# Hansard-T/FHE-Linformer

Hardware: AMD Instinct MI355X
Metric: encrypted Linformer-d128 forward ms/sample (lower is better)
Workload: dtype u64

## Files before the change

fhe-linformer_amd/csrc/context.cpp:

```cpp
#include "context.h"
#include <hip/hip_runtime.h>
#include <algorithm>
#include <cstdio>
#include <cstdlib>
#include <cstring>
#include <sys/random.h>
#include <time.h>
#include <cxxabi.h>
#include <dlfcn.h>
#include <execinfo.h>

namespace fhelin {

void hip_check(hipError_t e, const char* what) {
    if (e != hipSuccess) throw Error(FHELIN_ERR_HIP, std::string(what) + ": " + hipGetErrorString(e));
}

void* DevicePool::raw_malloc(size_t bytes) {
    if (backend_.malloc_fn) return backend_.malloc_fn(bytes);
    void* p = nullptr;
    if (hipMalloc(&p, bytes) != hipSuccess) {
        (void)hipGetLastError();
        return nullptr;
    }
// ... 279 lines not shown
            hip_check(hipStreamCreateWithFlags(&lane_stream[k], hipStreamNonBlocking), "hipStreamCreate(lane)");
            hip_check(hipEventCreateWithFlags(&lane_event[k], hipEventDisableTiming), "hipEventCreate(lane)");
        }
        hip_check(hipEventCreateWithFlags(&fork_event, hipEventDisableTiming), "hipEventCreate(fork)");
        pool.lane_stream[0] = main_stream;
        for (int k = 1; k <= n_lanes; ++k) pool.lane_stream[k] = lane_stream[k];
        pool.have_streams = true;
        if (const char* e = std::getenv("FHELIN_ASYNC")) async_lanes = std::atoi(e) != 0;
        if (const char* e = std::getenv("FHELIN_FUSE_MODDOWN")) fuse_moddown = std::atoi(e) != 0;
        if (const char* e = std::getenv("FHELIN_FUSE_FINISH")) fuse_finish = std::atoi(e) != 0;
        if (const char* e = std::getenv("FHELIN_HOST_ENCODE")) host_encode = std::atoi(e) != 0;
        if (const char* e = std::getenv("FHELIN_FUSE_GATHER")) fuse_gather = std::atoi(e) != 0;
        if (const char* e = std::getenv("FHELIN_ROT_GATHER")) rot_gather = std::atoi(e) != 0;
        if (const char* e = std::getenv("FHELIN_FUSE_LIFT")) fuse_lift = std::atoi(e) != 0;
        if (const char* e = std::getenv("FHELIN_LDS_DIGITS")) lds_digits = std::atoi(e) != 0;
        if (const char* e = std::getenv("FHELIN_NTT_TRACE")) trace_small_ntt = std::atoi(e);
        if (const char* e = std::getenv("FHELIN_SCALAR_TRACE")) trace_scalar = std::atoi(e);
        if (const char* e = std::getenv("FHELIN_HOST_WAITS")) trace_waits = std::atoi(e) != 0;
    }
    hip_check(hipEventCreate(&ev_start), "hipEventCreate");
    stage_words = (size_t)2 << p.log_n;
    for (int i = 0; i < STAGE_SLOTS; ++i) {
        hip_check(hipHostMalloc(reinterpret_cast<void**>(&stage_buf[i]), stage_words * sizeof(u64), hipHostMallocDefault), "hipHostMalloc(stage)");
        hip_check(hipEventCreateWithFlags(&stage_ev[i], hipEventDisableTiming), "hipEventCreate(stage)");
    }
    hip_check(hipHostMalloc(reinterpret_cast<void**>(&small_buf), (size_t)SMALL_SLOTS * SMALL_WORDS * sizeof(u64), hipHostMallocDefault), "hipHostMalloc(stage, small)");
    for (int i = 0; i < SMALL_SLOTS; ++i) hip_check(hipEventCreateWithFlags(&small_ev[i], hipEventDisableTiming), "hipEventCreate(stage, small)");
    hip_check(hipEventCreate(&ev_stop), "hipEventCreate");
    has_device = true;

// ... 375 lines not shown
```

fhe-linformer_amd/csrc/context.h:

```cpp
#pragma once
#include <cstdint>
#include <map>
#include <memory>
#include <stdexcept>
#include <string>
#include <unordered_map>
#include <vector>
#include <hip/hip_runtime_api.h>
#include "../../include/fhelin.h"
#include "hostmath.h"
#include "kernels.h"

namespace fhelin {

struct Params {
    int log_n = 16;
    int n_q = 24;
    int first_bits = 55;
    int scale_bits = 52;
    int n_p = 6;
    int special_bits = 60;
    int dnum = 4;
    int log_slots = 14;
    int hamming = 192;
// ... 204 lines not shown
    int limb_id_p(int j) const { return L + 1 + j; }
    int digits_at(int ell) const { return (ell + alpha - 1) / alpha; }
    u64 galois_element(int rot_index) const;
    const u32* automorph_map(u64 galois);
    const u32* automorph_inverse_of(const u32* map);
    std::map<const u32*, const u32*> automorph_inverse;
    u32 automorph_ginv_of(const u32* map) const;
    std::map<const u32*, u32> automorph_ginv;
    bool fuse_finish = true;
    bool fuse_moddown = false;
    bool host_encode = false;
    bool fuse_gather = true;
    bool rot_gather = true;
    bool fuse_lift = true;
    bool lds_digits = true;
    struct FftDev {
        const u32* rot = nullptr;
        const double* ksi = nullptr;
    };
    std::map<int, FftDev> fft_dev;
    void sync();
    void ntt(const LimbBatch& b, bool inverse, int active = -1) {
        stats.limb_ntt += (u64)(active >= 0 ? active : b.nvec);
        if (trace_small_ntt && b.nvec <= trace_small_ntt) note_small_ntt(b.nvec);
        launch_ntt(dt, b, inverse, stream);
    }
    bool trace_waits = false;
    std::map<std::string, std::pair<u64, u64>> wait_sites;
    void note_wait(const char* site, u64 ns) {
        auto& e = wait_sites[site];
// ... 18 lines not shown
```

fhe-linformer_amd/csrc/evaluator.cpp:

```cpp
#include "evaluator.h"
#include <map>
#include <hip/hip_runtime.h>
#include <cmath>
#include <cstring>

namespace fhelin {

DevBlock::~DevBlock() {
    if (d && ctx) {
        try { ctx->pool.free(d); } catch (...) {}
    }
}
Ciphertext::~Ciphertext() {
    if (async_ev) (void)hipEventDestroy(async_ev);
    if (d && ctx && !block) {
        try { ctx->pool.free(d); } catch (...) {}
    }
}
Encoding::~Encoding() {
    if (ready) (void)hipEventDestroy(ready);
    if (d && ctx) {
        try { ctx->pool.free(d, lanes_ordered); } catch (...) {}
    }
}
EvalKey::~EvalKey() {
    if (d && ctx) {
        try { ctx->pool.free(d); } catch (...) {}
    }
    if (d_perm && ctx) {
        try { ctx->pool.free(d_perm); } catch (...) {}
    }
}

static void launch_ok(const char* what) { hip_check(hipGetLastError(), what); }

CtPtr Evaluator::new_ct(int npoly, int ell, int deg, long double scale, int slots) {
    c_.require_device();
    if (ell < 1 || ell > c_.L + 1 || npoly < 1 || npoly > 3) throw Error(FHELIN_ERR_ARG, "new_ct: bad shape");
    auto ct = std::make_shared<Ciphertext>();
    ct->ctx = &c_;
    ct->npoly = npoly;
    ct->ell = ell;
    ct->deg = deg;
    ct->scale = scale;
    ct->slots = slots;
// ... 100 lines not shown
    if (rows) {
        sh.per_row = 1;
        sh.shared_input = shared ? 1 : 0;
        for (int b = 0; b < B; ++b) {
            sh.evk_row[b] = rows->keys[b]->d;
            sh.map_row[b] = rows->maps[b];
        }
    }
    KsShape shu = sh;
    shu.batch = shared ? 1 : B;
    c_.stats.keyswitch += (u64)B;
    c_.stats.keyswitch_limbs += (u64)B * ell;
    const bool identity = !map && !rows;
    const bool gather = !identity && !add1 && rot_in_gather();
    const u64* evk = key ? key->d : nullptr;
    if (gather) {
        sh.gather = 1;
        if (rows) {
            for (int b = 0; b < B; ++b) {
                sh.evk_row[b] = permuted(*rows->keys[b], rows->maps[b]);
                sh.ginv_row[b] = c_.automorph_ginv_of(rows->maps[b]);
            }
        } else {
            evk = permuted(*key, map);
            sh.map_row[0] = map;
            sh.ginv = c_.automorph_ginv_of(map);
        }
        if (add0) {
            sh.gsrc = add0;
            sh.gsrc_stride = add_stride;
// ... 130 lines not shown
        if (!rot_keys.count(c_.galois_element(r))) return false;
    }
    return !indices.empty();
}

const u64* Evaluator::permuted(const EvalKey& key, const u32* map) {
    if (key.d_perm) return key.d_perm;
    const int nvec = key.digits * 2 * (c_.L + 1 + c_.K);
    key.d_perm = c_.dalloc<u64>(key.words());
    launch_automorph_pack30(c_.dt, key.d_perm, key.d, map, nvec, c_.stream);
    launch_ok("key permutation");
    hip_check(hipStreamSynchronize(c_.stream), "key permutation sync");
    return key.d_perm;
}

std::vector<CtPtr> Evaluator::rotate_sum_batch(const std::vector<CtPtr>& vin, const std::vector<int>& indices) {
    if (vin.empty()) return {};
    const int R = (int)indices.size();
    if (R < 1 || R > KsShape::MAX_ROT) throw Error(FHELIN_ERR_ARG, "rotate_sum_batch: 1..7 rotations");
    if (!have_rotation_keys(indices, vin[0]->slots)) throw Error(FHELIN_ERR_KEY, "rotate_sum_batch: missing rotation key");
    if (c_.K < 1) throw Error(FHELIN_ERR_STATE, "hybrid key switching needs at least one special prime");
    std::vector<const EvalKey*> keys;
    std::vector<const u32*> maps;
    for (int r : indices) {
        const u64 g = c_.galois_element(r);
        keys.push_back(rot_keys.at(g).get());
        maps.push_back(c_.automorph_map(g));
    }
    const size_t N = c_.N;
    const int K = c_.K, L1 = c_.L + 1;
// ... 7 lines not shown
        for (size_t i = first; i < vin.size() && (int)idx.size() < batch_limit; ++i) {
            const CtPtr &a = vin[first], &b = vin[i];
            if (!done[i] && b->npoly == 2 && b->ell == a->ell && b->deg == a->deg && fabsl(b->scale / a->scale - 1.0L) < 1e-9L)
                idx.push_back(i);
        }
        std::vector<CtPtr> chunk;
        for (size_t i : idx) chunk.push_back(vin[i]);
        chunk = make_contiguous(chunk, 0);
        const int B = (int)chunk.size(), ell = chunk[0]->ell;
        const size_t pn = (size_t)ell * N, ctw = 2 * pn;
        const LevelTables& lt = c_.lvl[ell];
        std::vector<CtPtr> o = new_ct_batch(B, 2, ell, chunk[0]->deg, chunk[0]->scale, chunk[0]->slots);
        const u64* base = chunk[0]->d;
        KsShape sh{ell, K, c_.alpha, lt.beta, L1, B, ctw, ctw, pn, ctw};
        sh.n_rot = R;
        sh.lds_digits = c_.lds_digits ? 1 : 0;
        for (int r = 0; r < R; ++r) {
            sh.evk_rot[r] = permuted(*keys[r], maps[r]);
            sh.map_rot[r] = maps[r];
            if (c_.galois_element(indices[r]) % (u64)(c_.N / 256) != 1) sh.lds_digits = 0;
        }
        int steps = 0;
        while ((1 << steps) < R + 1) ++steps;
        c_.stats.keyswitch += (u64)B * steps;
        c_.stats.keyswitch_limbs += (u64)B * steps * ell;
        {
            Scratch<u64> ext = modup(sh, base + pn, false);
            Scratch<u64> accQ = c_.scratch<u64>((size_t)B * 2 * ell * N);
            Scratch<u64> accP = c_.scratch<u64>((size_t)B * 2 * K * N);
            const bool rp = sum_in_row_pass();
            if (c_.fuse_gather) {
// ... 100 lines not shown
        }
        std::vector<CtPtr> chunk;
        for (size_t i : idx) chunk.push_back(x[i]);
        chunk = make_contiguous(chunk, 0);
        const int B = (int)chunk.size(), ell = chunk[0]->ell;
        const size_t pn = (size_t)ell * N, ctw = 2 * pn;
        const LevelTables& lt = c_.lvl[ell];
        const long double sf = c_.sf_real[chunk[0]->level()];
        const bool merged = rescale_out && ell >= 2 && K + 1 <= 16;
        if (rescale_out && !merged) throw Error(FHELIN_ERR_STATE, "hoisted_dot_rows: no limb left to drop");
        const int oell = merged ? ell - 1 : ell;
        std::vector<CtPtr> o = new_ct_batch(B, 2, oell, merged ? chunk[0]->deg : chunk[0]->deg + 1, chunk[0]->scale * sf, chunk[0]->slots);
        const u64* base = chunk[0]->d;
        KsShape sh{ell, K, c_.alpha, lt.beta, L1, B, ctw, (size_t)2 * oell * N, pn, ctw};
        sh.n_rot = R;
        sh.lds_digits = c_.lds_digits ? 1 : 0;
        HoistAdd h;
        h.n_rot = R;
        std::vector<FoldedKey> hold;
        const std::shared_ptr<Encoding> e0 = pts[0]->at(ell, sf);
        h.v[0] = e0->d;
        for (int r = 0; r < R; ++r) {
            hold.push_back(folded_key(pts[r + 1], indices[r], sf));
            sh.evk_rot[r] = hold.back().d->d;
            sh.map_rot[r] = maps[r];
            h.v[r + 1] = hold.back().enc->d;
            h.map[r] = maps[r];
            if (c_.galois_element(indices[r]) % (u64)(c_.N / 256) != 1) sh.lds_digits = 0;
        }
        c_.stats.keyswitch += (u64)B * R;
        c_.stats.keyswitch_limbs += (u64)B * R * ell;
// ... 1054 lines not shown
            sadj = make_contiguous(sadj, 7);
        }
        ScalarSet cst;
        if (cadd != 0.0) real_to_scalars(c_, (long double)cadd * sc, ell, cst);
        KsShape sh{ell, K, c_.alpha, lt.beta, L1, B, 3 * pn, (size_t)2 * (ell - 1) * N, pn, 0};
        c_.stats.keyswitch += (u64)B;
        c_.stats.keyswitch_limbs += (u64)B * ell;
        c_.stats.rescale += (u64)B;
        c_.stats.rescale_limbs += (u64)B * ell;
        const u64* c_ntt = d[0]->d + 2 * pn;
        std::vector<CtPtr> o = new_ct_batch(B, 2, ell - 1, 1, 0, x[first]->slots);
        {
            Scratch<u64> ext = modup(sh, c_ntt, true);
            Scratch<u64> accQ = c_.scratch<u64>((size_t)B * 2 * ell * N);
            Scratch<u64> accP = c_.scratch<u64>((size_t)B * 2 * K * N);
            launch_ks_inner(c_.dt, sh, accQ, accP, ext, relin_key->d, c_ntt, s);
            launch_affine_acc(c_.dt, sh, accQ, d[0]->d, sadj.empty() ? nullptr : sadj[0]->d, cst, cadd != 0.0 ? 1 : 0, f, c_.d_pmod, s);
            if (f == 2) launch_ew_add(c_.dt, accP, accP, accP, B * 2 * K, B * 2 * K, L1, K, s);
            moddown_rescale(sh, accQ, accP, o[0]->d);
            launch_ok("mult_affine_rescale_batch");
        }
        for (int k = 0; k < B; ++k) {
            const size_t i = idx[k];
            o[k]->scale = x[i]->scale * y[i]->scale / (long double)c_.chain.q[ell - 1];
            out[i] = o[k];
            done[i] = 1;
        }
    }
    return out;
}

// ... 98 lines not shown
        }
        Scratch<u64> dcst = c_.scratch<u64>(cst.size());
        if (items.cst) c_.upload_async(dcst, cst.data(), cst.size());
        KsShape sh{ell, K, c_.alpha, c_.lvl[ell].beta, L1, B, 3 * pn, (size_t)2 * (ell - 1) * N, pn, 0};
        sh.accp_limbs = K + 1;
        c_.stats.keyswitch += (u64)B;
        c_.stats.keyswitch_limbs += (u64)B * ell;
        c_.stats.rescale += (u64)B;
        c_.stats.rescale_limbs += (u64)B * ell;
        const u64* c_ntt = d[0]->d + 2 * pn;
        std::vector<CtPtr> o = new_ct_batch(B, 2, ell - 1, 1, 0, x[first]->slots);
        {
            Scratch<u64> ext = modup(sh, c_ntt, true);
            Scratch<u64> accQ = c_.scratch<u64>((size_t)B * 2 * ell * N);
            Scratch<u64> accP = c_.scratch<u64>((size_t)B * 2 * (K + 1) * N);
            launch_ks_inner(c_.dt, sh, accQ, accP, ext, relin_key->d, c_ntt, s);
            launch_affine_acc_items(c_.dt, sh, items, accQ, accP, d[0]->d, dcst, c_.d_pmod, s);
            moddown_rescale_exact(sh, accQ, accP, o[0]->d, items.f2);
            launch_ok("mult_affine_batch");
        }
        for (int k = 0; k < B; ++k) {
            const size_t i = idx[k];
            o[k]->scale = x[i]->scale * y[i]->scale / (long double)c_.chain.q[ell - 1];
            out[i] = o[k];
            done[i] = 1;
        }
    }
    return out;
}

std::vector<CtPtr> Evaluator::add_plain_batch(const std::vector<CtPtr>& v, const PtPtr& p) {
    std::vector<CtPtr> out(v.size());
// ... 391 lines not shown
```

fhe-linformer_amd/csrc/evaluator.h:

```cpp
#pragma once
#include <functional>
#include <map>
#include <memory>
#include <vector>
#include "context.h"
#include "kernels_elem.h"

namespace fhelin {

struct DevBlock {
    Context* ctx = nullptr;
    u64* d = nullptr;
    ~DevBlock();
};

struct Ciphertext {
    Context* ctx = nullptr;
    u64* d = nullptr;
    std::shared_ptr<DevBlock> block;
    int npoly = 2;
    int ell = 0;
    int deg = 1;
    long double scale = 0;
    int slots = 0;
// ... 30 lines not shown
    std::vector<double> imag;
    int slots = 0;
    int level = 0;
    static constexpr size_t MAX_ENCODINGS = 16;
    std::vector<std::shared_ptr<Encoding>> cache;
    std::shared_ptr<Encoding> at(int ell, long double scale);
    std::shared_ptr<Plaintext> shared;
    static constexpr size_t MAX_SHARED_ENCODINGS = 64;
};
typedef std::shared_ptr<Plaintext> PtPtr;

struct EvalKey {
    Context* ctx = nullptr;
    u64* d = nullptr;
    mutable u64* d_perm = nullptr;
    int digits = 0;
    bool seeded = false;
    ~EvalKey();
    size_t words() const { return (size_t)digits * 2 * (ctx->L + 1 + ctx->K) * ctx->N; }
};
typedef std::shared_ptr<EvalKey> KeyPtr;

void real_to_scalars(const Context& c, long double v, int ell, ScalarSet& sc);

class Evaluator {
public:
    explicit Evaluator(Context& c) : c_(c) {}
    Context& ctx() { return c_; }

    CtPtr new_ct(int npoly, int ell, int deg, long double scale, int slots);
// ... 16 lines not shown

    void keyswitch(const u64* c_ntt, int ell, const EvalKey& key, u64* out, const u64* add0, const u64* add1, const u32* map,
                   const u64* post = nullptr);
    void keyswitch_batch(int batch, const u64* c_ntt, size_t c_stride, int ell, const EvalKey& key, u64* out, size_t out_stride,
                         const u64* add0, const u64* add1, size_t add_stride, const u32* map, const u64* post, size_t post_stride);
    struct KsRows {
        std::vector<const EvalKey*> keys;
        std::vector<const u32*> maps;
        bool shared_input = false;
    };
    void keyswitch_rows(const KsRows& rows, const u64* c_ntt, size_t c_stride, int ell, u64* out, size_t out_stride, const u64* add0,
                        size_t add_stride);
    std::vector<CtPtr> rotate_sum_batch(const std::vector<CtPtr>& v, const std::vector<int>& indices);
    bool have_rotation_keys(const std::vector<int>& indices, int slots) const;
    const u64* permuted(const EvalKey& key, const u32* map);
    CtPtr rotate_each_sum(const std::vector<CtPtr>& v, const std::vector<int>& indices);
    std::vector<CtPtr> rotate_each_sum_rows(const std::vector<std::vector<CtPtr>>& rows, const std::vector<int>& indices);
    std::vector<CtPtr> hoisted_dot_rows(const std::vector<CtPtr>& xs, const std::vector<PtPtr>& pts, const std::vector<int>& indices,
                                        bool rescale_out = false);
    bool merged_products = false;
    bool merged_rescale = true;
    bool double_hoist = true;
    struct FoldedKey {
        PtPtr pt;
        KeyPtr key;
        int index = 0;
        long double scale = 0;
        std::shared_ptr<Encoding> enc;
        std::shared_ptr<DevBlock> d;
    };
// ... 101 lines not shown
```

fhe-linformer_amd/csrc/kernels_elem.h:

```cpp
#pragma once
#include "kernels.h"

namespace fhelin {

struct ScalarSet {
    u64 v[128];
};

void launch_ew_mul(const DeviceTables& t, u64* out, const u64* a, const u64* b, int nvec, int b_mod, int limb_first, int limb_count, hipStream_t s);
void launch_ew_add(const DeviceTables& t, u64* out, const u64* a, const u64* b, int nvec, int b_mod, int limb_first, int limb_count, hipStream_t s);
void launch_ew_sub(const DeviceTables& t, u64* out, const u64* a, const u64* b, int nvec, int b_mod, int limb_first, int limb_count, hipStream_t s);
void launch_ew_muladd(const DeviceTables& t, u64* out, const u64* acc, const u64* a, const u64* b, int nvec, int b_mod, int limb_first,
                      int limb_count, hipStream_t s);
void launch_ew_neg(const DeviceTables& t, u64* out, const u64* a, int nvec, int limb_first, int limb_count, hipStream_t s);
void launch_ew_scalar(const DeviceTables& t, u64* out, const u64* a, const ScalarSet& sc, int nvec, int limb_first, int limb_count, hipStream_t s,
                      int in_limbs = 0);
void launch_ew_addscalar(const DeviceTables& t, u64* out, const u64* a, const ScalarSet& sc, int nvec, int limb_first, int limb_count, hipStream_t s,
                         int add_vecs = -1);
struct LinComb {
    static constexpr int MAX_TERMS = 32;
    int n = 0;
    int vecs = 0;
    const u64* a[MAX_TERMS];
};
// ... 101 lines not shown
    int n_rot = 0;
    const u64* evk_rot[MAX_ROT] = {};
    const u32* map_rot[MAX_ROT] = {};
    size_t rot_ext_stride = 0;
    size_t rot_input_stride = 0;
    int lds_digits = 0;
    size_t ext_batch_stride = 0;
    const u64* gsrc = nullptr;
    size_t gsrc_stride = 0;
    const u64* gsrc_pmod = nullptr;
    int gather = 0;
    u32 ginv = 0;
    u32 ginv_row[MAX_ROWS] = {};
    int tch = 16;
    int accp_limbs = 0;
};
void launch_modup_conv(const DeviceTables& t, const KsShape& sh, u64* ext, const u64* cc, const u64* c_ntt, const u64* hatinv,
                       const u64* hatmod, hipStream_t s);
void launch_ks_inner(const DeviceTables& t, const KsShape& sh, u64* accQ, u64* accP, const u64* ext, const u64* evk, const u64* c_ntt,
                     hipStream_t s);
void launch_ks_inner_multi(const DeviceTables& t, const KsShape& sh, u64* accQ, u64* accP, const u64* ext, const u64* c_ntt,
                           hipStream_t s);
void launch_fold_key(const DeviceTables& t, u64* out, const u64* key, const u32* map, const u64* V, int nvec, hipStream_t s);
struct HoistAdd {
    int n_rot = 0;
    const u64* v[KsShape::MAX_ROT + 1] = {};
    const u32* map[KsShape::MAX_ROT] = {};
    u64* acc = nullptr;
    const u64* pmod = nullptr;
};
void launch_hoist_addends(const DeviceTables& t, const KsShape& sh, const HoistAdd& h, u64* pre, const u64* ct, hipStream_t s);
void launch_gather_sum(const DeviceTables& t, const KsShape& sh, u64* out, const u64* in, size_t in_stride, hipStream_t s);
void launch_moddown_conv(const DeviceTables& t, const KsShape& sh, u64* conv, const u64* accP, const u64* phatinv, const u64* phatmod,
                         hipStream_t s);
void launch_affine_acc(const DeviceTables& t, const KsShape& sh, u64* accQ, const u64* d, const u64* sub, const ScalarSet& cst, int has_cst, int f,
                       const u64* pmod, hipStream_t s);
void launch_moddown_rescale_conv(const DeviceTables& t, const KsShape& sh, u64* conv, const u64* accP, const u64* top, const u64* hatinv,
                                 const u64* hatmod, const u64* mmod, hipStream_t s);
void launch_moddown_rescale_finish(const DeviceTables& t, const KsShape& sh, u64* out, const u64* accQ, const u64* conv, const u64* minv,
                                   hipStream_t s);
struct AffineItems {
    static constexpr int MAX_ITEMS = 32;
    const u64* add[MAX_ITEMS] = {};
    u32 f2 = 0, neg = 0, cst = 0;
};
void launch_affine_acc_items(const DeviceTables& t, const KsShape& sh, const AffineItems& it, u64* accQ, u64* accP, const u64* d,
                             const u64* consts, const u64* pmod, hipStream_t s);
void launch_moddown_rescale_exact_conv(const DeviceTables& t, const KsShape& sh, u32 f2, u64* conv, const u64* accP, const u64* phatinv,
                                       const u64* phatmod, const u64* pinv, const u64* pmod, const u64* qlm, hipStream_t s);
void launch_moddown_finish(const DeviceTables& t, const KsShape& sh, u64* out, const u64* accQ, const u64* conv, const u64* pinv,
                           const u64* add0, const u64* add1, const u32* map, const u64* post, hipStream_t s);

}
```

fhe-linformer_amd/csrc/kernels_ks.hip:

```cpp
#include <hip/hip_runtime.h>
#include <cstdlib>
#include "kernels.h"
#include "kernels_elem.h"

namespace fhelin {
namespace {

typedef u64 u64x2 __attribute__((ext_vector_type(2)));

__device__ __forceinline__ Barrett load_barrett(const DeviceTables& t, int limb) {
    Barrett b;
    b.q = t.moduli[limb];
    b.r0 = t.barrett[2 * limb];
    b.r1 = t.barrett[2 * limb + 1];
    return b;
}

constexpr int TCH = 16;

template <int MAXA, bool FULL>
__device__ __forceinline__ void modup_body(const DeviceTables& t, const KsShape& sh, u64* __restrict__ ext, const u64* __restrict__ cc,
                                           const u64* __restrict__ hatinv, const u64* __restrict__ hatmod, int j, int lo, int cnt, size_t n) {
    const size_t N = (size_t)1 << t.log_n;
    const int nt = sh.ell + sh.k;
// ... 56 lines not shown
    unsigned b = blockIdx.y * nx + blockIdx.x;
    if ((nblk & 7) == 0) b = (b & 7) * (nblk >> 3) + (b >> 3);
    KsBlock k;
    k.bi = (int)(b % nb);
    k.bx = (int)((b / nb) % nx);
    k.tt = (int)(b / (nb * nx));
    return k;
}

__device__ __forceinline__ u32 sel_mask(u32 a, u32 b, unsigned long long mask) {
    u32 r;
    asm("v_cndmask_b32_e64 %0, %1, %2, %3" : "=v"(r) : "v"(a), "v"(b), "s"(mask));
    return r;
}

template <bool GATHER>
__global__ __launch_bounds__(256) void ks_inner_kernel(DeviceTables t, KsShape sh, u64* __restrict__ accQ, u64* __restrict__ accP, const u64* __restrict__ ext,
                                                       const u64* __restrict__ evk, const u64* __restrict__ c_ntt) {
    const int nt = sh.ell + sh.k;
    const KsBlock kb_ = ks_block(sh);
    const int bi = kb_.bi, tt = kb_.tt;
    const int limb = tt < sh.ell ? tt : sh.L1 + (tt - sh.ell);
    const int in = sh.row_mod ? bi / sh.row_mod : bi;
    const int ri = sh.per_row ? (sh.row_mod ? bi % sh.row_mod : bi) : 0;
    if (sh.row_mod) {
        ext += (size_t)in * sh.ext_batch_stride;
        c_ntt += (size_t)in * sh.c_stride;
        evk = sh.evk_row[bi % sh.row_mod];
    } else {
        if (!sh.shared_input) {
            ext += (size_t)bi * sh.beta * nt * ((size_t)1 << t.log_n);
            c_ntt += (size_t)bi * sh.c_stride;
        }
// ... 28 lines not shown
            const u64x2 ka = K[(size_t)(2 * j + 1) * kstride + (size_t)limb * row + n2];
            if constexpr (GATHER) {
                u32 p0, p1, q0, q1;
                split30(d.x, p0, p1);
                split30(d.y, q0, q1);
                const u32 dx0 = sel_mask(p0, q0, swp), dx1 = sel_mask(p1, q1, swp), dy0 = sel_mask(q0, p0, swp), dy1 = sel_mask(q1, p1, swp);
                mac30(b0, dx0, dx1, (u32)kb.x, (u32)(kb.x >> 32));
                mac30(b1, dy0, dy1, (u32)kb.y, (u32)(kb.y >> 32));
                mac30(a0, dx0, dx1, (u32)ka.x, (u32)(ka.x >> 32));
                mac30(a1, dy0, dy1, (u32)ka.y, (u32)(ka.y >> 32));
            } else {
                if (j == own) {
                    d.x = mul_shoup(d.x, monR, monRs, br.q);
                    d.y = mul_shoup(d.y, monR, monRs, br.q);
                }
                u32 dx0, dx1, dy0, dy1, k0, k1;
                split30(d.x, dx0, dx1);
                split30(d.y, dy0, dy1);
                split30(kb.x, k0, k1);
                mac30(b0, dx0, dx1, k0, k1);
                split30(kb.y, k0, k1);
                mac30(b1, dy0, dy1, k0, k1);
                split30(ka.x, k0, k1);
                mac30(a0, dx0, dx1, k0, k1);
                split30(ka.y, k0, k1);
                mac30(a1, dy0, dy1, k0, k1);
            }
        }
        acc30_flush(b0, lo[0], hi[0]);
        acc30_flush(b1, lo[1], hi[1]);
        acc30_flush(a0, lo[2], hi[2]);
        acc30_flush(a1, lo[3], hi[3]);
    }
    u64x2 rb, ra;
    const u64 qi = t.qinv[limb];
    rb.x = redc128(lo[0], hi[0], br.q, qi);
    rb.y = redc128(lo[1], hi[1], br.q, qi);
    ra.x = redc128(lo[2], hi[2], br.q, qi);
    ra.y = redc128(lo[3], hi[3], br.q, qi);
    if (tt < sh.ell) {
        if constexpr (GATHER) {
            if (sh.gsrc_pmod) {
                const u64x2 gp = reinterpret_cast<const u64x2*>(sh.gsrc + (size_t)in * sh.gsrc_stride)[(size_t)tt * row + nd];
                const u64 w = sh.gsrc_pmod[2 * tt], ws = sh.gsrc_pmod[2 * tt + 1];
                rb.x = add_mod(rb.x, mul_shoup((m0 & 1) ? gp.y : gp.x, w, ws, br.q), br.q);
                rb.y = add_mod(rb.y, mul_shoup((m0 & 1) ? gp.x : gp.y, w, ws, br.q), br.q);
            }
        }
        u64x2* O = reinterpret_cast<u64x2*>(accQ);
        O[(size_t)tt * row + n2] = rb;
        O[(size_t)(sh.ell + tt) * row + n2] = ra;
    } else {
        u64x2* O = reinterpret_cast<u64x2*>(accP);
        const int pj = tt - sh.ell;
        O[(size_t)pj * row + n2] = rb;
        O[(size_t)(pk + pj) * row + n2] = ra;
    }
}

template <bool STAGE, int ROWS>
__global__ __launch_bounds__(256) void ks_inner_multi_kernel(DeviceTables t, KsShape sh, u64* __restrict__ accQ, u64* __restrict__ accP,
                                                             const u64* __restrict__ ext, const u64* __restrict__ c_ntt) {
    __shared__ u64x2 dl[STAGE ? ROWS : 1][STAGE ? 4 : 1][256];
    const int nt = sh.ell + sh.k;
    const KsBlock kb_ = ks_block(sh, (sh.batch + ROWS - 1) / ROWS);
    const int bi = kb_.bi * ROWS, tt = kb_.tt;
    const int limb = tt < sh.ell ? tt : sh.L1 + (tt - sh.ell);
    const size_t N = (size_t)1 << t.log_n, row = N >> 1;
    const size_t ext_stride = sh.ext_batch_stride ? sh.ext_batch_stride : (size_t)sh.beta * nt * N;
    const int own = tt < sh.ell ? tt / sh.alpha : -1;
    const Barrett br = load_barrett(t, limb);
    const size_t n2 = (size_t)kb_.bx * 256 + threadIdx.x;
    const size_t kstride = (size_t)(sh.L1 + sh.k) * row;
    bool live[ROWS];
    const u64* extr[ROWS];
// ... 8 lines not shown
    u64 lo[ROWS][4], hi[ROWS][4];
    Acc30 acc[ROWS][4];
#pragma unroll
    for (int q = 0; q < ROWS; ++q)
#pragma unroll
        for (int i = 0; i < 4; ++i) {
            lo[q][i] = hi[q][i] = 0;
            acc[q][i] = Acc30{0, 0, 0};
        }
    int pending = 0, folded = 0;
    if constexpr (STAGE) {
#pragma unroll
        for (int q = 0; q < ROWS; ++q) {
            const u64x2* __restrict__ e0 = reinterpret_cast<const u64x2*>(extr[q]);
            const u64x2* __restrict__ c0 = reinterpret_cast<const u64x2*>(cr_[q]);
            for (int j = 0; j < sh.beta; ++j) dl[q][j][threadIdx.x] = j == own ? c0[(size_t)tt * row + n2] : e0[((size_t)j * nt + tt) * row + n2];
        }
        __syncthreads();
    }
    struct Operands {
        u64x2 d[ROWS], kb, ka;
    };
    auto map_of = [&](int r) -> u32 { return sh.map_rot[r] ? sh.map_rot[r][2 * n2] : (u32)(2 * n2); };
    auto issue = [&](int r, int j, u32 m0) {
        const size_t mp = m0 >> 1;
        const u64x2* __restrict__ K = reinterpret_cast<const u64x2*>(sh.evk_rot[r]) + (size_t)limb * row + n2;
        Operands o;
#pragma unroll
        for (int q = 0; q < ROWS; ++q) {
            if constexpr (STAGE) {
                o.d[q] = dl[q][j][mp & 255];
// ... 21 lines not shown
        }
        Operands nxt = cur;
        if (it + 1 < total) {
            nxt = issue(rn, jn, mn);
            if (jn == 0 && rn + 1 < sh.n_rot) m_nxt = map_of(rn + 1);
        }
        {
            const unsigned long long swp = __ballot((m_cur & 1) != 0);
            const u64x2 kb = cur.kb, ka = cur.ka;
            const u32 kbx0 = (u32)kb.x, kbx1 = (u32)(kb.x >> 32), kby0 = (u32)kb.y, kby1 = (u32)(kb.y >> 32);
            const u32 kax0 = (u32)ka.x, kax1 = (u32)(ka.x >> 32), kay0 = (u32)ka.y, kay1 = (u32)(ka.y >> 32);
#pragma unroll
            for (int q = 0; q < ROWS; ++q) {
                const u64x2 d = cur.d[q];
                u32 p0, p1, q0, q1;
                split30(d.x, p0, p1);
                split30(d.y, q0, q1);
                const u32 dx0 = sel_mask(p0, q0, swp), dx1 = sel_mask(p1, q1, swp), dy0 = sel_mask(q0, p0, swp), dy1 = sel_mask(q1, p1, swp);
                mac30(acc[q][0], dx0, dx1, kbx0, kbx1);
                mac30(acc[q][1], dy0, dy1, kby0, kby1);
                mac30(acc[q][2], dx0, dx1, kax0, kax1);
                mac30(acc[q][3], dy0, dy1, kay0, kay1);
            }
            if (++pending == 8) {
                pending = 0;
                const bool fold = ++folded == 2;
                if (fold) folded = 0;
#pragma unroll
                for (int q = 0; q < ROWS; ++q)
#pragma unroll
                    for (int i = 0; i < 4; ++i) {
                        acc30_flush(acc[q][i], lo[q][i], hi[q][i]);
// ... 181 lines not shown
    }
    if (sh.gsrc && !sh.gsrc_pmod && c == 0) {
        const u64* __restrict__ g = sh.gsrc + (size_t)bi * sh.gsrc_stride + (size_t)tt * N;
        for (int rr = 0; rr < sh.n_rot; ++rr) {
            const u64* __restrict__ gr = g + (size_t)rr * sh.rot_input_stride;
            const u32* __restrict__ mr = sh.map_rot[rr];
            const u32 m0 = mr ? mr[j] : (u32)j;
            const u64x2 gp = reinterpret_cast<const u64x2*>(gr)[m0 >> 1];
            r.x = add_mod(r.x, (m0 & 1) ? gp.y : gp.x, q);
            r.y = add_mod(r.y, (m0 & 1) ? gp.x : gp.y, q);
        }
    }
    reinterpret_cast<u64x2*>(out)[((size_t)v * N + j) >> 1] = r;
}

__global__ __launch_bounds__(256) void fold_key_kernel(DeviceTables t, u64* __restrict__ out, const u64* __restrict__ key, const u32* __restrict__ map,
                                                       const u64* __restrict__ V) {
    const size_t v = blockIdx.y;
    const int limb = (int)(v % (size_t)t.n_limbs);
    const Barrett br = load_barrett(t, limb);
    const size_t N = (size_t)1 << t.log_n;
    const size_t j = ((size_t)blockIdx.x * 256 + threadIdx.x) * 2;
    const u32 m0 = map[j], m1 = map[j + 1];
    const u64x2 pv = reinterpret_cast<const u64x2*>(V)[((size_t)limb * N + j) >> 1];
    u64x2 r;
    const u64 R = t.mont[2 * limb], Rs = t.mont[2 * limb + 1];
    r.x = pack30(mul_shoup(mul_mod(pv.x, key[v * N + m0], br), R, Rs, br.q));
    r.y = pack30(mul_shoup(mul_mod(pv.y, key[v * N + m1], br), R, Rs, br.q));
    reinterpret_cast<u64x2*>(out)[(v * N + j) >> 1] = r;
}
// ... 104 lines not shown
                }
            acc30_flush(acc, slo, shi);
        }
        dst[(size_t)tt * N] = sub_mod(barrett_reduce128(slo, shi, br), barrett_reduce128((u64)neg * mmod[tt], 0, br), br.q);
    }
}

__global__ __launch_bounds__(256) void affine_acc_items_kernel(DeviceTables t, KsShape sh, AffineItems it, u64* __restrict__ accQ, u64* __restrict__ accP,
                                                               const u64* __restrict__ d, const u64* __restrict__ consts, const u64* __restrict__ pmod) {
    const int bi = blockIdx.y / (2 * sh.ell), v = blockIdx.y % (2 * sh.ell);
    const int c = v / sh.ell, tt = v % sh.ell;
    const bool f2 = (it.f2 >> bi) & 1;
    const size_t row = ((size_t)1 << t.log_n) >> 1;
    const size_t n2 = (size_t)blockIdx.x * 256 + threadIdx.x;
    const u64 q = t.moduli[tt];
    u64x2 x = reinterpret_cast<const u64x2*>(d)[(((size_t)bi * 3 + c) * sh.ell + tt) * row + n2];
    if (f2) {
        x.x = add_mod(x.x, x.x, q);
        x.y = add_mod(x.y, x.y, q);
    }
    if (c == 0 && ((it.cst >> bi) & 1)) {
        const u64 k = consts[(size_t)bi * sh.ell + tt];
        x.x = add_mod(x.x, k, q);
        x.y = add_mod(x.y, k, q);
    }
    const u64* __restrict__ add = it.add[bi];
    if (add) {
        const u64x2 sv = reinterpret_cast<const u64x2*>(add)[((size_t)c * sh.ell + tt) * row + n2];
        if ((it.neg >> bi) & 1) {
            x.x = sub_mod(x.x, sv.x, q);
            x.y = sub_mod(x.y, sv.y, q);
        } else {
            x.x = add_mod(x.x, sv.x, q);
            x.y = add_mod(x.y, sv.y, q);
        }
    }
    u64x2* A = reinterpret_cast<u64x2*>(accQ) + (((size_t)bi * 2 + c) * sh.ell + tt) * row + n2;
    u64x2 a = *A;
    if (f2) {
        a.x = add_mod(a.x, a.x, q);
        a.y = add_mod(a.y, a.y, q);
    }
    const u64 w = pmod[2 * tt], ws = pmod[2 * tt + 1];
    a.x = add_mod(a.x, mul_shoup(x.x, w, ws, q), q);
    a.y = add_mod(a.y, mul_shoup(x.y, w, ws, q), q);
    if (tt == sh.ell - 1)
        reinterpret_cast<u64x2*>(accP)[(((size_t)bi * 2 + c) * (sh.k + 1) + sh.k) * row + n2] = a;
    else
        *A = a;
}

template <int MAXK, bool FULL>
__device__ __forceinline__ void moddown_exact_body(const DeviceTables& t, const KsShape& sh, bool f2, u64* __restrict__ dst, const u64* __restrict__ src,
                                                   const u64* __restrict__ phatinv, const u64* __restrict__ phatmod, const u64* __restrict__ pinv,
                                                   const u64* __restrict__ pmod, const u64* __restrict__ qlm) {
    const size_t N = (size_t)1 << t.log_n;
    u32 z0[MAXK], z1[MAXK];
#pragma unroll
    for (int p = 0; p < MAXK; ++p) {
        if (FULL || p < sh.k) {
// ... 124 lines not shown
void launch_modup_conv(const DeviceTables& t, const KsShape& sh_in, u64* ext, const u64* cc, const u64* c_ntt, const u64* hatinv,
                       const u64* hatmod, hipStream_t s) {
    KsShape sh = sh_in;
    const unsigned nx = (1u << t.log_n) / 256;
    sh.tch = conv_tch(nx * (unsigned)(sh.batch * sh.beta), sh.ell + sh.k);
    dim3 g(nx, (unsigned)(sh.batch * sh.beta), (unsigned)((sh.ell + sh.k + sh.tch - 1) / sh.tch));
#define FHELIN_MODUP_CASE(A) case A: hipLaunchKernelGGL((modup_conv_kernel<A>), g, dim3(256), 0, s, t, sh, ext, cc, c_ntt, hatinv, hatmod); break;
    switch (sh.alpha) {
        FHELIN_MODUP_CASE(1) FHELIN_MODUP_CASE(2) FHELIN_MODUP_CASE(3) FHELIN_MODUP_CASE(4)
        FHELIN_MODUP_CASE(5) FHELIN_MODUP_CASE(6) FHELIN_MODUP_CASE(7) FHELIN_MODUP_CASE(8)
        default: hipLaunchKernelGGL((modup_conv_kernel<16>), g, dim3(256), 0, s, t, sh, ext, cc, c_ntt, hatinv, hatmod); break;
    }
#undef FHELIN_MODUP_CASE
}
void launch_ks_inner(const DeviceTables& t, const KsShape& sh, u64* accQ, u64* accP, const u64* ext, const u64* evk, const u64* c_ntt,
                     hipStream_t s) {
    dim3 g((1u << t.log_n) / 512, (unsigned)(sh.batch * (sh.ell + sh.k)));
    if (sh.gather)
        hipLaunchKernelGGL(ks_inner_kernel<true>, g, dim3(256), 0, s, t, sh, accQ, accP, ext, evk, c_ntt);
    else
        hipLaunchKernelGGL(ks_inner_kernel<false>, g, dim3(256), 0, s, t, sh, accQ, accP, ext, evk, c_ntt);
}
void launch_ks_inner_multi(const DeviceTables& t, const KsShape& sh, u64* accQ, u64* accP, const u64* ext, const u64* c_ntt,
                           hipStream_t s) {
    static const int pair_rows = [] { const char* e = std::getenv("FHELIN_KS_ROW_PAIRS"); return e ? std::atoi(e) : 1; }();
    const bool stage = sh.lds_digits && sh.rot_ext_stride == 0 && sh.beta <= 4;
    if (pair_rows && sh.batch >= 2) {
        dim3 g((1u << t.log_n) / 512, (unsigned)(((sh.batch + 1) / 2) * (sh.ell + sh.k)));
        if (stage)
            hipLaunchKernelGGL((ks_inner_multi_kernel<true, 2>), g, dim3(256), 0, s, t, sh, accQ, accP, ext, c_ntt);
        else
            hipLaunchKernelGGL((ks_inner_multi_kernel<false, 2>), g, dim3(256), 0, s, t, sh, accQ, accP, ext, c_ntt);
        return;
    }
    dim3 g((1u << t.log_n) / 512, (unsigned)(sh.batch * (sh.ell + sh.k)));
    if (stage)
        hipLaunchKernelGGL((ks_inner_multi_kernel<true, 1>), g, dim3(256), 0, s, t, sh, accQ, accP, ext, c_ntt);
    else
        hipLaunchKernelGGL((ks_inner_multi_kernel<false, 1>), g, dim3(256), 0, s, t, sh, accQ, accP, ext, c_ntt);
}
void launch_gather_sum(const DeviceTables& t, const KsShape& sh, u64* out, const u64* in, size_t in_stride, hipStream_t s) {
    dim3 g((1u << t.log_n) / 256, (unsigned)(sh.batch * sh.ell));
    hipLaunchKernelGGL(gather_sum_kernel, g, dim3(256), 0, s, t, sh, out, in, in_stride);
}
void launch_moddown_conv(const DeviceTables& t, const KsShape& sh_in, u64* conv, const u64* accP, const u64* phatinv, const u64* phatmod,
                         hipStream_t s) {
    KsShape sh = sh_in;
    const unsigned nx = (1u << t.log_n) / 256;
    sh.tch = conv_tch(nx * (unsigned)(2 * sh.batch), sh.ell);
    dim3 g(nx, (unsigned)(2 * sh.batch), (unsigned)((sh.ell + sh.tch - 1) / sh.tch));
#define FHELIN_MODDOWN_CASE(K, S) case K: hipLaunchKernelGGL((moddown_conv_kernel<K, S>), g, dim3(256), 0, s, t, sh, conv, accP, phatinv, phatmod); break;
// ... 22 lines not shown
```

Measured before the change: 226.9.

## Fuse affine step into key-switch inner product and pre-split relin key and staged digits

Adds three default-on options. The affine accumulation in mult_affine_batch now runs inside the ks_inner kernel, which removes a separate launch and a read-modify-write pass over accQ. The relinearization key is repacked once into 30-bit halves so the inner loop skips split30 on key words. The rotation multi-kernel also pre-splits digits when staging them into LDS, so split30 runs once per digit rather than on every reuse. The costs are an extra persistent device copy of the relin key, a one-time synchronous pack pass, and more kernel template variants.

```diff
diff --git a/fhe-linformer_amd/csrc/context.cpp b/fhe-linformer_amd/csrc/context.cpp
--- a/fhe-linformer_amd/csrc/context.cpp
+++ b/fhe-linformer_amd/csrc/context.cpp
@@ -317,6 +317,9 @@
         if (const char* e = std::getenv("FHELIN_ROT_GATHER")) rot_gather = std::atoi(e) != 0;
         if (const char* e = std::getenv("FHELIN_FUSE_LIFT")) fuse_lift = std::atoi(e) != 0;
         if (const char* e = std::getenv("FHELIN_LDS_DIGITS")) lds_digits = std::atoi(e) != 0;
+        if (const char* e = std::getenv("FHELIN_FUSE_AFFINE")) fuse_affine = std::atoi(e) != 0;
+        if (const char* e = std::getenv("FHELIN_PRESPLIT_RELIN")) presplit_relin = std::atoi(e) != 0;
+        if (const char* e = std::getenv("FHELIN_STAGE_HALVES")) stage_halves = std::atoi(e) != 0;
         if (const char* e = std::getenv("FHELIN_NTT_TRACE")) trace_small_ntt = std::atoi(e);
         if (const char* e = std::getenv("FHELIN_SCALAR_TRACE")) trace_scalar = std::atoi(e);
         if (const char* e = std::getenv("FHELIN_HOST_WAITS")) trace_waits = std::atoi(e) != 0;
diff --git a/fhe-linformer_amd/csrc/context.h b/fhe-linformer_amd/csrc/context.h
--- a/fhe-linformer_amd/csrc/context.h
+++ b/fhe-linformer_amd/csrc/context.h
@@ -242,6 +242,9 @@
     bool rot_gather = true;
     bool fuse_lift = true;
     bool lds_digits = true;
+    bool fuse_affine = true;
+    bool presplit_relin = true;
+    bool stage_halves = true;
     struct FftDev {
         const u32* rot = nullptr;
         const double* ksi = nullptr;
diff --git a/fhe-linformer_amd/csrc/evaluator.cpp b/fhe-linformer_amd/csrc/evaluator.cpp
--- a/fhe-linformer_amd/csrc/evaluator.cpp
+++ b/fhe-linformer_amd/csrc/evaluator.cpp
@@ -29,6 +29,9 @@
     }
     if (d_perm && ctx) {
         try { ctx->pool.free(d_perm); } catch (...) {}
+    }
+    if (d_split && ctx) {
+        try { ctx->pool.free(d_split); } catch (...) {}
     }
 }
 
@@ -159,6 +162,10 @@
     const bool identity = !map && !rows;
     const bool gather = !identity && !add1 && rot_in_gather();
     const u64* evk = key ? key->d : nullptr;
+    if (!gather && key) {
+        evk = relin_words(*key);
+        sh.evk_split = evk != key->d;
+    }
     if (gather) {
         sh.gather = 1;
         if (rows) {
@@ -319,6 +326,16 @@
     return key.d_perm;
 }
 
+const u64* Evaluator::relin_words(const EvalKey& key) {
+    if (!c_.presplit_relin || &key != relin_key.get()) return key.d;
+    if (key.d_split) return key.d_split;
+    key.d_split = c_.dalloc<u64>(key.words());
+    launch_pack30(c_.dt, key.d_split, key.d, key.digits * 2 * (c_.L + 1 + c_.K), c_.stream);
+    launch_ok("key split");
+    hip_check(hipStreamSynchronize(c_.stream), "key split sync");
+    return key.d_split;
+}
+
 std::vector<CtPtr> Evaluator::rotate_sum_batch(const std::vector<CtPtr>& vin, const std::vector<int>& indices) {
     if (vin.empty()) return {};
     const int R = (int)indices.size();
@@ -356,7 +373,7 @@
         const u64* base = chunk[0]->d;
         KsShape sh{ell, K, c_.alpha, lt.beta, L1, B, ctw, ctw, pn, ctw};
         sh.n_rot = R;
-        sh.lds_digits = c_.lds_digits ? 1 : 0;
+        sh.lds_digits = c_.lds_digits ? (c_.stage_halves ? 2 : 1) : 0;
         for (int r = 0; r < R; ++r) {
             sh.evk_rot[r] = permuted(*keys[r], maps[r]);
             sh.map_rot[r] = maps[r];
@@ -487,7 +504,7 @@
         const u64* base = chunk[0]->d;
         KsShape sh{ell, K, c_.alpha, lt.beta, L1, B, ctw, (size_t)2 * oell * N, pn, ctw};
         sh.n_rot = R;
-        sh.lds_digits = c_.lds_digits ? 1 : 0;
+        sh.lds_digits = c_.lds_digits ? (c_.stage_halves ? 2 : 1) : 0;
         HoistAdd h;
         h.n_rot = R;
         std::vector<FoldedKey> hold;
@@ -1572,7 +1589,9 @@
             Scratch<u64> ext = modup(sh, c_ntt, true);
             Scratch<u64> accQ = c_.scratch<u64>((size_t)B * 2 * ell * N);
             Scratch<u64> accP = c_.scratch<u64>((size_t)B * 2 * K * N);
-            launch_ks_inner(c_.dt, sh, accQ, accP, ext, relin_key->d, c_ntt, s);
+            const u64* evk = relin_words(*relin_key);
+            sh.evk_split = evk != relin_key->d;
+            launch_ks_inner(c_.dt, sh, accQ, accP, ext, evk, c_ntt, s);
             launch_affine_acc(c_.dt, sh, accQ, d[0]->d, sadj.empty() ? nullptr : sadj[0]->d, cst, cadd != 0.0 ? 1 : 0, f, c_.d_pmod, s);
             if (f == 2) launch_ew_add(c_.dt, accP, accP, accP, B * 2 * K, B * 2 * K, L1, K, s);
             moddown_rescale(sh, accQ, accP, o[0]->d);
@@ -1701,8 +1720,19 @@
             Scratch<u64> ext = modup(sh, c_ntt, true);
             Scratch<u64> accQ = c_.scratch<u64>((size_t)B * 2 * ell * N);
             Scratch<u64> accP = c_.scratch<u64>((size_t)B * 2 * (K + 1) * N);
-            launch_ks_inner(c_.dt, sh, accQ, accP, ext, relin_key->d, c_ntt, s);
-            launch_affine_acc_items(c_.dt, sh, items, accQ, accP, d[0]->d, dcst, c_.d_pmod, s);
+            const u64* evk = relin_words(*relin_key);
+            sh.evk_split = evk != relin_key->d;
+            if (c_.fuse_affine) {
+                KsAffine aff;
+                aff.it = items;
+                aff.d = d[0]->d;
+                aff.consts = dcst;
+                aff.pmod = c_.d_pmod;
+                launch_ks_inner(c_.dt, sh, accQ, accP, ext, evk, c_ntt, s, &aff);
+            } else {
+                launch_ks_inner(c_.dt, sh, accQ, accP, ext, evk, c_ntt, s);
+                launch_affine_acc_items(c_.dt, sh, items, accQ, accP, d[0]->d, dcst, c_.d_pmod, s);
+            }
             moddown_rescale_exact(sh, accQ, accP, o[0]->d, items.f2);
             launch_ok("mult_affine_batch");
         }
diff --git a/fhe-linformer_amd/csrc/evaluator.h b/fhe-linformer_amd/csrc/evaluator.h
--- a/fhe-linformer_amd/csrc/evaluator.h
+++ b/fhe-linformer_amd/csrc/evaluator.h
@@ -68,6 +68,7 @@
     Context* ctx = nullptr;
     u64* d = nullptr;
     mutable u64* d_perm = nullptr;
+    mutable u64* d_split = nullptr;
     int digits = 0;
     bool seeded = false;
     ~EvalKey();
@@ -114,6 +115,7 @@
     std::vector<CtPtr> rotate_sum_batch(const std::vector<CtPtr>& v, const std::vector<int>& indices);
     bool have_rotation_keys(const std::vector<int>& indices, int slots) const;
     const u64* permuted(const EvalKey& key, const u32* map);
+    const u64* relin_words(const EvalKey& key);
     CtPtr rotate_each_sum(const std::vector<CtPtr>& v, const std::vector<int>& indices);
     std::vector<CtPtr> rotate_each_sum_rows(const std::vector<std::vector<CtPtr>>& rows, const std::vector<int>& indices);
     std::vector<CtPtr> hoisted_dot_rows(const std::vector<CtPtr>& xs, const std::vector<PtPtr>& pts, const std::vector<int>& indices,
diff --git a/fhe-linformer_amd/csrc/kernels_elem.h b/fhe-linformer_amd/csrc/kernels_elem.h
--- a/fhe-linformer_amd/csrc/kernels_elem.h
+++ b/fhe-linformer_amd/csrc/kernels_elem.h
@@ -139,11 +139,14 @@
     u32 ginv_row[MAX_ROWS] = {};
     int tch = 16;
     int accp_limbs = 0;
+    int evk_split = 0;
 };
 void launch_modup_conv(const DeviceTables& t, const KsShape& sh, u64* ext, const u64* cc, const u64* c_ntt, const u64* hatinv,
                        const u64* hatmod, hipStream_t s);
+struct KsAffine;
 void launch_ks_inner(const DeviceTables& t, const KsShape& sh, u64* accQ, u64* accP, const u64* ext, const u64* evk, const u64* c_ntt,
-                     hipStream_t s);
+                     hipStream_t s, const KsAffine* aff = nullptr);
+void launch_pack30(const DeviceTables& t, u64* out, const u64* key, int nvec, hipStream_t s);
 void launch_ks_inner_multi(const DeviceTables& t, const KsShape& sh, u64* accQ, u64* accP, const u64* ext, const u64* c_ntt,
                            hipStream_t s);
 void launch_fold_key(const DeviceTables& t, u64* out, const u64* key, const u32* map, const u64* V, int nvec, hipStream_t s);
@@ -169,6 +172,12 @@
     const u64* add[MAX_ITEMS] = {};
     u32 f2 = 0, neg = 0, cst = 0;
 };
+struct KsAffine {
+    AffineItems it;
+    const u64* d = nullptr;
+    const u64* consts = nullptr;
+    const u64* pmod = nullptr;
+};
 void launch_affine_acc_items(const DeviceTables& t, const KsShape& sh, const AffineItems& it, u64* accQ, u64* accP, const u64* d,
                              const u64* consts, const u64* pmod, hipStream_t s);
 void launch_moddown_rescale_exact_conv(const DeviceTables& t, const KsShape& sh, u32 f2, u64* conv, const u64* accP, const u64* phatinv,
diff --git a/fhe-linformer_amd/csrc/kernels_ks.hip b/fhe-linformer_amd/csrc/kernels_ks.hip
--- a/fhe-linformer_amd/csrc/kernels_ks.hip
+++ b/fhe-linformer_amd/csrc/kernels_ks.hip
@@ -1,5 +1,6 @@
 #include <hip/hip_runtime.h>
 #include <cstdlib>
+#include <type_traits>
 #include "kernels.h"
 #include "kernels_elem.h"
 
@@ -94,9 +95,42 @@
     return r;
 }
 
-template <bool GATHER>
-__global__ __launch_bounds__(256) void ks_inner_kernel(DeviceTables t, KsShape sh, u64* __restrict__ accQ, u64* __restrict__ accP, const u64* __restrict__ ext,
-                                                       const u64* __restrict__ evk, const u64* __restrict__ c_ntt) {
+__device__ __forceinline__ u64x2 affine_item(u64x2 a, u64x2 x, bool f2, bool has_cst, u64 cst, const u64x2* __restrict__ addend, bool neg,
+                                             u64 w, u64 ws, u64 q) {
+    if (f2) {
+        x.x = add_mod(x.x, x.x, q);
+        x.y = add_mod(x.y, x.y, q);
+    }
+    if (has_cst) {
+        x.x = add_mod(x.x, cst, q);
+        x.y = add_mod(x.y, cst, q);
+    }
+    if (addend) {
+        const u64x2 sv = *addend;
+        if (neg) {
+            x.x = sub_mod(x.x, sv.x, q);
+            x.y = sub_mod(x.y, sv.y, q);
+        } else {
+            x.x = add_mod(x.x, sv.x, q);
+            x.y = add_mod(x.y, sv.y, q);
+        }
+    }
+    if (f2) {
+        a.x = add_mod(a.x, a.x, q);
+        a.y = add_mod(a.y, a.y, q);
+    }
+    a.x = add_mod(a.x, mul_shoup(x.x, w, ws, q), q);
+    a.y = add_mod(a.y, mul_shoup(x.y, w, ws, q), q);
+    return a;
+}
+
+struct NoAffine {};
+
+template <bool GATHER, bool SPLIT, class AFF>
+__global__ __launch_bounds__(256) void ks_inner_kernel(DeviceTables t, KsShape sh, AFF aff, u64* __restrict__ accQ, u64* __restrict__ accP,
+                                                       const u64* __restrict__ ext, const u64* __restrict__ evk, const u64* __restrict__ c_ntt) {
+    constexpr bool AFFINE = !std::is_same<AFF, NoAffine>::value;
+    static_assert(!(GATHER && (SPLIT || AFFINE)), "the gathered inner product has its own key copy and no affine step");
     const int nt = sh.ell + sh.k;
     const KsBlock kb_ = ks_block(sh);
     const int bi = kb_.bi, tt = kb_.tt;
@@ -155,17 +189,25 @@
                     d.x = mul_shoup(d.x, monR, monRs, br.q);
                     d.y = mul_shoup(d.y, monR, monRs, br.q);
                 }
-                u32 dx0, dx1, dy0, dy1, k0, k1;
+                u32 dx0, dx1, dy0, dy1;
+                [[maybe_unused]] u32 k0, k1;
                 split30(d.x, dx0, dx1);
                 split30(d.y, dy0, dy1);
-                split30(kb.x, k0, k1);
-                mac30(b0, dx0, dx1, k0, k1);
-                split30(kb.y, k0, k1);
-                mac30(b1, dy0, dy1, k0, k1);
-                split30(ka.x, k0, k1);
-                mac30(a0, dx0, dx1, k0, k1);
-                split30(ka.y, k0, k1);
-                mac30(a1, dy0, dy1, k0, k1);
+                if constexpr (SPLIT) {
+                    mac30(b0, dx0, dx1, (u32)kb.x, (u32)(kb.x >> 32));
+                    mac30(b1, dy0, dy1, (u32)kb.y, (u32)(kb.y >> 32));
+                    mac30(a0, dx0, dx1, (u32)ka.x, (u32)(ka.x >> 32));
+                    mac30(a1, dy0, dy1, (u32)ka.y, (u32)(ka.y >> 32));
+                } else {
+                    split30(kb.x, k0, k1);
+                    mac30(b0, dx0, dx1, k0, k1);
+                    split30(kb.y, k0, k1);
+                    mac30(b1, dy0, dy1, k0, k1);
+                    split30(ka.x, k0, k1);
+                    mac30(a0, dx0, dx1, k0, k1);
+                    split30(ka.y, k0, k1);
+                    mac30(a1, dy0, dy1, k0, k1);
+                }
             }
         }
         acc30_flush(b0, lo[0], hi[0]);
@@ -188,6 +230,22 @@
                 rb.y = add_mod(rb.y, mul_shoup((m0 & 1) ? gp.x : gp.y, w, ws, br.q), br.q);
             }
         }
+        if constexpr (AFFINE) {
+            const bool f2 = (aff.it.f2 >> bi) & 1, neg = (aff.it.neg >> bi) & 1, has_cst = (aff.it.cst >> bi) & 1;
+            const u64 cst = has_cst ? aff.consts[(size_t)bi * sh.ell + tt] : 0;
+            const u64 w = aff.pmod[2 * tt], ws = aff.pmod[2 * tt + 1];
+            const u64x2* D = reinterpret_cast<const u64x2*>(aff.d) + ((size_t)bi * 3 * sh.ell + tt) * row + n2;
+            const u64x2* A = reinterpret_cast<const u64x2*>(aff.it.add[bi]);
+            if (A) A += (size_t)tt * row + n2;
+            rb = affine_item(rb, D[0], f2, has_cst, cst, A, neg, w, ws, br.q);
+            ra = affine_item(ra, D[(size_t)sh.ell * row], f2, false, 0, A ? A + (size_t)sh.ell * row : A, neg, w, ws, br.q);
+            if (tt == sh.ell - 1) {
+                u64x2* O = reinterpret_cast<u64x2*>(accP);
+                O[(size_t)sh.k * row + n2] = rb;
+                O[(size_t)(pk + sh.k) * row + n2] = ra;
+                return;
+            }
+        }
         u64x2* O = reinterpret_cast<u64x2*>(accQ);
         O[(size_t)tt * row + n2] = rb;
         O[(size_t)(sh.ell + tt) * row + n2] = ra;
@@ -199,7 +257,7 @@
     }
 }
 
-template <bool STAGE, int ROWS>
+template <bool STAGE, int ROWS, bool HALVES = false>
 __global__ __launch_bounds__(256) void ks_inner_multi_kernel(DeviceTables t, KsShape sh, u64* __restrict__ accQ, u64* __restrict__ accP,
                                                              const u64* __restrict__ ext, const u64* __restrict__ c_ntt) {
     __shared__ u64x2 dl[STAGE ? ROWS : 1][STAGE ? 4 : 1][256];
@@ -238,7 +296,14 @@
         for (int q = 0; q < ROWS; ++q) {
             const u64x2* __restrict__ e0 = reinterpret_cast<const u64x2*>(extr[q]);
             const u64x2* __restrict__ c0 = reinterpret_cast<const u64x2*>(cr_[q]);
-            for (int j = 0; j < sh.beta; ++j) dl[q][j][threadIdx.x] = j == own ? c0[(size_t)tt * row + n2] : e0[((size_t)j * nt + tt) * row + n2];
+            for (int j = 0; j < sh.beta; ++j) {
+                u64x2 v = j == own ? c0[(size_t)tt * row + n2] : e0[((size_t)j * nt + tt) * row + n2];
+                if constexpr (HALVES) {
+                    v.x = pack30(v.x);
+                    v.y = pack30(v.y);
+                }
+                dl[q][j][threadIdx.x] = v;
+            }
         }
         __syncthreads();
     }
@@ -290,8 +355,12 @@
             for (int q = 0; q < ROWS; ++q) {
                 const u64x2 d = cur.d[q];
                 u32 p0, p1, q0, q1;
-                split30(d.x, p0, p1);
-                split30(d.y, q0, q1);
+                if constexpr (HALVES) {
+                    p0 = (u32)d.x, p1 = (u32)(d.x >> 32), q0 = (u32)d.y, q1 = (u32)(d.y >> 32);
+                } else {
+                    split30(d.x, p0, p1);
+                    split30(d.y, q0, q1);
+                }
                 const u32 dx0 = sel_mask(p0, q0, swp), dx1 = sel_mask(p1, q1, swp), dy0 = sel_mask(q0, p0, swp), dy1 = sel_mask(q1, p1, swp);
                 mac30(acc[q][0], dx0, dx1, kbx0, kbx1);
                 mac30(acc[q][1], dy0, dy1, kby0, kby1);
@@ -503,6 +572,14 @@
     reinterpret_cast<u64x2*>(out)[((size_t)v * N + j) >> 1] = r;
 }
 
+__global__ __launch_bounds__(256) void pack30_kernel(int log_n, u64* __restrict__ out, const u64* __restrict__ key) {
+    const size_t i = (size_t)blockIdx.y * (((size_t)1 << log_n) >> 1) + (size_t)blockIdx.x * 256 + threadIdx.x;
+    u64x2 r = reinterpret_cast<const u64x2*>(key)[i];
+    r.x = pack30(r.x);
+    r.y = pack30(r.y);
+    reinterpret_cast<u64x2*>(out)[i] = r;
+}
+
 __global__ __launch_bounds__(256) void fold_key_kernel(DeviceTables t, u64* __restrict__ out, const u64* __restrict__ key, const u32* __restrict__ map,
                                                        const u64* __restrict__ V) {
     const size_t v = blockIdx.y;
@@ -637,36 +714,13 @@
     const size_t row = ((size_t)1 << t.log_n) >> 1;
     const size_t n2 = (size_t)blockIdx.x * 256 + threadIdx.x;
     const u64 q = t.moduli[tt];
-    u64x2 x = reinterpret_cast<const u64x2*>(d)[(((size_t)bi * 3 + c) * sh.ell + tt) * row + n2];
-    if (f2) {
-        x.x = add_mod(x.x, x.x, q);
-        x.y = add_mod(x.y, x.y, q);
-    }
-    if (c == 0 && ((it.cst >> bi) & 1)) {
-        const u64 k = consts[(size_t)bi * sh.ell + tt];
-        x.x = add_mod(x.x, k, q);
-        x.y = add_mod(x.y, k, q);
-    }
-    const u64* __restrict__ add = it.add[bi];
-    if (add) {
-        const u64x2 sv = reinterpret_cast<const u64x2*>(add)[((size_t)c * sh.ell + tt) * row + n2];
-        if ((it.neg >> bi) & 1) {
-            x.x = sub_mod(x.x, sv.x, q);
-            x.y = sub_mod(x.y, sv.y, q);
-        } else {
-            x.x = add_mod(x.x, sv.x, q);
-            x.y = add_mod(x.y, sv.y, q);
-        }
-    }
+    const u64x2 x = reinterpret_cast<const u64x2*>(d)[(((size_t)bi * 3 + c) * sh.ell + tt) * row + n2];
+    const bool has_cst = c == 0 && ((it.cst >> bi) & 1);
+    const u64 k = has_cst ? consts[(size_t)bi * sh.ell + tt] : 0;
+    const u64x2* add = reinterpret_cast<const u64x2*>(it.add[bi]);
+    if (add) add += ((size_t)c * sh.ell + tt) * row + n2;
     u64x2* A = reinterpret_cast<u64x2*>(accQ) + (((size_t)bi * 2 + c) * sh.ell + tt) * row + n2;
-    u64x2 a = *A;
-    if (f2) {
-        a.x = add_mod(a.x, a.x, q);
-        a.y = add_mod(a.y, a.y, q);
-    }
-    const u64 w = pmod[2 * tt], ws = pmod[2 * tt + 1];
-    a.x = add_mod(a.x, mul_shoup(x.x, w, ws, q), q);
-    a.y = add_mod(a.y, mul_shoup(x.y, w, ws, q), q);
+    const u64x2 a = affine_item(*A, x, f2, has_cst, k, add, (it.neg >> bi) & 1, pmod[2 * tt], pmod[2 * tt + 1], q);
     if (tt == sh.ell - 1)
         reinterpret_cast<u64x2*>(accP)[(((size_t)bi * 2 + c) * (sh.k + 1) + sh.k) * row + n2] = a;
     else
@@ -821,27 +875,42 @@
 #undef FHELIN_MODUP_CASE
 }
 void launch_ks_inner(const DeviceTables& t, const KsShape& sh, u64* accQ, u64* accP, const u64* ext, const u64* evk, const u64* c_ntt,
-                     hipStream_t s) {
+                     hipStream_t s, const KsAffine* aff) {
     dim3 g((1u << t.log_n) / 512, (unsigned)(sh.batch * (sh.ell + sh.k)));
+    const NoAffine none;
     if (sh.gather)
-        hipLaunchKernelGGL(ks_inner_kernel<true>, g, dim3(256), 0, s, t, sh, accQ, accP, ext, evk, c_ntt);
+        hipLaunchKernelGGL((ks_inner_kernel<true, false, NoAffine>), g, dim3(256), 0, s, t, sh, none, accQ, accP, ext, evk, c_ntt);
+    else if (aff && sh.evk_split)
+        hipLaunchKernelGGL((ks_inner_kernel<false, true, KsAffine>), g, dim3(256), 0, s, t, sh, *aff, accQ, accP, ext, evk, c_ntt);
+    else if (aff)
+        hipLaunchKernelGGL((ks_inner_kernel<false, false, KsAffine>), g, dim3(256), 0, s, t, sh, *aff, accQ, accP, ext, evk, c_ntt);
+    else if (sh.evk_split)
+        hipLaunchKernelGGL((ks_inner_kernel<false, true, NoAffine>), g, dim3(256), 0, s, t, sh, none, accQ, accP, ext, evk, c_ntt);
     else
-        hipLaunchKernelGGL(ks_inner_kernel<false>, g, dim3(256), 0, s, t, sh, accQ, accP, ext, evk, c_ntt);
+        hipLaunchKernelGGL((ks_inner_kernel<false, false, NoAffine>), g, dim3(256), 0, s, t, sh, none, accQ, accP, ext, evk, c_ntt);
+}
+void launch_pack30(const DeviceTables& t, u64* out, const u64* key, int nvec, hipStream_t s) {
+    hipLaunchKernelGGL(pack30_kernel, dim3((1u << t.log_n) / 512, (unsigned)nvec), dim3(256), 0, s, t.log_n, out, key);
 }
 void launch_ks_inner_multi(const DeviceTables& t, const KsShape& sh, u64* accQ, u64* accP, const u64* ext, const u64* c_ntt,
                            hipStream_t s) {
     static const int pair_rows = [] { const char* e = std::getenv("FHELIN_KS_ROW_PAIRS"); return e ? std::atoi(e) : 1; }();
     const bool stage = sh.lds_digits && sh.rot_ext_stride == 0 && sh.beta <= 4;
+    const bool halves = stage && sh.lds_digits == 2;
     if (pair_rows && sh.batch >= 2) {
         dim3 g((1u << t.log_n) / 512, (unsigned)(((sh.batch + 1) / 2) * (sh.ell + sh.k)));
-        if (stage)
+        if (halves)
+            hipLaunchKernelGGL((ks_inner_multi_kernel<true, 2, true>), g, dim3(256), 0, s, t, sh, accQ, accP, ext, c_ntt);
+        else if (stage)
             hipLaunchKernelGGL((ks_inner_multi_kernel<true, 2>), g, dim3(256), 0, s, t, sh, accQ, accP, ext, c_ntt);
         else
             hipLaunchKernelGGL((ks_inner_multi_kernel<false, 2>), g, dim3(256), 0, s, t, sh, accQ, accP, ext, c_ntt);
         return;
     }
     dim3 g((1u << t.log_n) / 512, (unsigned)(sh.batch * (sh.ell + sh.k)));
-    if (stage)
+    if (halves)
+        hipLaunchKernelGGL((ks_inner_multi_kernel<true, 1, true>), g, dim3(256), 0, s, t, sh, accQ, accP, ext, c_ntt);
+    else if (stage)
         hipLaunchKernelGGL((ks_inner_multi_kernel<true, 1>), g, dim3(256), 0, s, t, sh, accQ, accP, ext, c_ntt);
     else
         hipLaunchKernelGGL((ks_inner_multi_kernel<false, 1>), g, dim3(256), 0, s, t, sh, accQ, accP, ext, c_ntt);
```

New measurement: 226.3 (median of 5 runs). About the same (-0.2%).
